# awslabs/flowgger

Hardware: AMD Instinct MI355X
Metric: log lines/sec (RFC5424, 256B avg) at 1/2/4/8 MI355X; achieved HBM GB/s (higher is better)
Workload: dtype u8

## Files before the change

### flowgger_amd/_lib.py

```python
from __future__ import annotations

import ctypes as C
from pathlib import Path

import os

_HERE = Path(__file__).resolve().parent
_ALT = os.environ.get("FLOWGGER_AMD_LIB") or ""
if _ALT and (Path(_ALT).name != _ALT or not _ALT.startswith("libfg_hip") or not _ALT.endswith(".so")):
    raise RuntimeError(f"FLOWGGER_AMD_LIB={_ALT!r}: only a bare libfg_hip*.so file name beside flowgger_amd/_lib.py is accepted")
LIB_PATH = _HERE / (_ALT or ("libfg_hip_prof.so" if os.environ.get("FLOWGGER_AMD_PROF_LIB") else "libfg_hip.so"))

FG_ABI_VERSION = 4
FG_RFC5424, FG_LTSV, FG_GELF, FG_RFC3164, FG_CAPNP = 0, 1, 2, 3, 4
FG_EF_VAL_ESC, FG_EF_NAME_ESC, FG_EF_SUFFIX, FG_EF_NAME_VERBATIM = 1, 2, 4, 8
FG_FRAME_NONE, FG_FRAME_LINE, FG_FRAME_NUL, FG_FRAME_SYSLEN = 0, 1, 2, 3
FG_SYSLEN_CLEAN, FG_SYSLEN_TAIL, FG_SYSLEN_BAD_LEN, FG_SYSLEN_LONG_PREFIX = 0, 1, 2, 3
FG_SYSLEN_MAX_PREFIX = 24
FG_UDP_RAW, FG_UDP_ZLIB, FG_UDP_GZIP, FG_UDP_BAD_ZLIB, FG_UDP_BAD_GZIP, FG_UDP_BAD_UTF8, FG_UDP_TOO_LARGE = range(7)
FG_UDP_DEFAULT_MAX_INFLATED = 65_527 * 5
FG_ST_OVERFLOW, FG_ST_BAD_UTF8 = 0xFE, 0xFD
FG_F_LTSV_NOVALUE = 128
FG_OK, FG_ERR_ARG, FG_ERR_HIP, FG_ERR_NO_DEVICE, FG_ERR_ENT_OVERFLOW, FG_ERR_UNSUPPORTED, FG_ERR_NOMEM = 0, -1, -2, -3, -4, -5, -6
FG_YEAR_NOW = -2147483648
# ... 45 lines not shown

class fg_launch_opts(C.Structure):
    _fields_ = [("lines_per_group", C.c_uint32), ("tile_cap", C.c_uint32), ("waves_per_cu", C.c_uint32),
                ("gelf_lds_budget", C.c_uint32), ("gelf_window_kib", C.c_uint32), ("flags", C.c_uint32), ("chunk_lines", C.c_uint32), ("ent_chunk", C.c_uint32), ("fused_look", C.c_uint32), ("fused_ext", C.c_uint32)]


FG_LO_GELF_GENERIC, FG_LO_TRANSCODE_ONE_PIECE, FG_LO_NO_HEAD, FG_LO_FORCE_HEAD, FG_LO_SD_WALK, FG_LO_SD_PAIRS, FG_LO_NO_ZERO_COPY, FG_LO_FRAME_KERNEL_UPLOAD = 1, 2, 4, 8, 16, 32, 64, 128
FG_LO_FRAME_CLASSIC = 256
FG_LO_STATIC_CHUNKS = 512
FG_LO_FRAME_SELFTEST_STALL = 1024
FG_LO_NO_TAPER = 2048
FG_LO_TAPER_1 = 4096
FG_LO_TAPER_2 = 8192
FG_LO_NO_FUSED_FRAMING = 16384
FG_LO_RFC3164_REGROUP, FG_LO_RFC3164_NO_REGROUP = 32768, 65536
FG_PATH_DECODE_ZERO_COPY, FG_PATH_DECODE_SLICED, FG_PATH_FRAME_FUSED, FG_PATH_FRAME_SLICED, FG_PATH_FRAME_ONE_PIECE = 1, 2, 3, 4, 5
FG_PATH_FRAME_SYSLEN_DEVICE, FG_PATH_FRAME_SYSLEN_HOST = 6, 7
FG_LO_RESERVED = 0x40000000


class fg_transcoded(C.Structure):
    _fields_ = [("out", C.c_void_p), ("out_bytes", C.c_uint64), ("out_offsets", C.c_void_p), ("meta", C.c_void_p),
                ("enc_status", C.c_void_p), ("frame_offsets", C.c_void_p), ("n", C.c_uint64), ("consumed", C.c_uint64)]


class fg_tz_table(C.Structure):
    _fields_ = [("n_zones", C.c_uint32), ("names", C.POINTER(C.c_char_p)), ("zone_first", C.c_void_p), ("utc_start", C.c_void_p),
                ("utc_offset", C.c_void_p)]


# ... 96 lines not shown
```

### flowgger_amd/csrc/fg_pipeline.hpp

```cpp
#pragma once
#include "fg_device.hpp"
#include "fg_plan_policy.hpp"
#include "fg_wave.hpp"

namespace fg {

using u32x4 = unsigned int __attribute__((ext_vector_type(4)));

__device__ __forceinline__ uint32_t eq_flags(uint32_t x, uint32_t pat) {
    uint32_t s = ((x & 0x7F7F7F7Fu) ^ pat) + 0x7F7F7F7Fu;
    return ~(s | x) & 0x80808080u;
}
__device__ __forceinline__ uint32_t range_flags(uint32_t x) {
    uint32_t l = x & 0x7F7F7F7Fu;
    uint32_t ge33 = l + 0x5F5F5F5Fu;
    uint32_t le126 = l + 0x01010101u;
    return ge33 & ~le126 & ~x & 0x80808080u;
}
__device__ __forceinline__ uint32_t ctrl_flags(uint32_t x) {
    uint32_t ge32 = (x & 0x7F7F7F7Fu) + 0x60606060u;
    return ~(ge32 | x) & 0x80808080u;
}
__device__ __forceinline__ uint32_t gather16(uint32_t f0, uint32_t f1, uint32_t f2, uint32_t f3) {
    uint32_t lo = __builtin_amdgcn_udot4(f1, 0x80402010u, __builtin_amdgcn_udot4(f0, 0x08040201u, 0u, false), false);
// ... 237 lines not shown
    return make_uint4(v.x, v.y, v.z, v.w);
#else
    return *p;
#endif
}

template <class F, class = void>
struct tail_batch { static constexpr int value = 4; };
template <class F>
struct tail_batch<F, decltype((void)F::kTailBatch)> { static constexpr int value = F::kTailBatch; };

template <class F, class = void>
struct defer_row_store { static constexpr bool value = true; };
template <class F>
struct defer_row_store<F, decltype((void)F::kDeferRowStore)> { static constexpr bool value = F::kDeferRowStore; };

constexpr uint32_t kHeadCap = 1024;
template <class F, class = void>
struct head_cap { static constexpr uint32_t value = kHeadCap; };
template <class F>
struct head_cap<F, decltype((void)F::kHeadBytes)> { static constexpr uint32_t value = F::kHeadBytes; };

template <int NB, bool PROF, class F, bool HEAD = false>
__device__ __forceinline__ void persistent_loop(const uint8_t* __restrict__ bytes, const uint64_t* __restrict__ offsets,
                                                uint64_t n, const DevTables& t, uint32_t tile_cap, uint32_t L, uint64_t chunk_lines,
                                                unsigned long long* prof, uint64_t* stash_base, F& fmt, FrameArgs fr) {
    static_assert(!HEAD || F::kClasses <= 1, "HEAD staging classifies one stage-A byte class at most");
    const uint64_t kChunkLines = chunk_lines;
    extern __shared__ __attribute__((aligned(16))) uint8_t smem[];
    uint16_t* bm16 = reinterpret_cast<uint16_t*>(smem + tile_cap + 64u);
// ... 281 lines not shown
                if (HEAD && e1 != o1) {
                    l2 = 0u;
                    if (e1 - o0 >= 1u) l2 = byte_at(e1 - 1);
                    if (e1 - o0 >= 2u) l2 |= byte_at(e1 - 2) << 8;
                }
            }
            GroupCtx c{bytes, smem, bm16, o0, e1, a0, span, valid, li, (ablate & 8u) ? nullptr : stash, ablate, ent_state, PROF ? prof + 6 : nullptr};
            c.tile_cap = tile_cap;
            if constexpr (HEAD) {
                const uint32_t al = (uint32_t)(o0 & 15ull), len = (uint32_t)(e1 - o0);
                c.tbase = tb + al;
                c.tlen = st == 0u ? 0u : (st - al < len ? st - al : len);
                c.last2 = l2;
            }
            pend = fmt.decode(c, t);
            if (fr.line_bad && valid && fr.line_bad[li]) {
                pend.meta = FG_ST_BAD_UTF8 | (0xFFu << 8) | (0xFFu << 16);
                pend.ts = 0.0;
#pragma unroll
                for (int k = 0; k < 6; ++k) pend.span[k] = fg_span{0, FG_NONE};
                pend.count = 0;
            }
            pend_li = li;
            pend_valid = valid;
#if defined(FG_ROW64_AB) && FG_ROW64_AB == 2
            pend_p = p;
            pend_nl = nl;
            if (!HEAD && defer_row_store<F>::value) {
                uint4 w[4];
                pack_row64(pend, w);
// ... 36 lines not shown
    }
#if defined(FG_ROW64_AB) && FG_ROW64_AB == 2
    if (!HEAD && defer_row_store<F>::value) {
        if (pend_valid && !(ablate & 1u)) {
            uint4* g = reinterpret_cast<uint4*>(t.meta) + pend_li * 4u;
            g[0] = pw0, g[1] = pw1, g[2] = pw2, g[3] = pw3;
        }
    } else if (pend_valid && !(ablate & 1u)) {
        store_row64_lane(t, pend_li, pend);
    }
#elif defined(FG_ROW64_AB)
    if (pend_valid && !(ablate & 1u)) store_row64_lane(t, pend_li, pend);
#else
    if (pend_valid && !(ablate & 1u)) store_row(t, pend_li, pend);
#endif
    if (PROF && lane == 0) {
        atomicAdd(&prof[0], (unsigned long long)acc0);
        atomicAdd(&prof[1], (unsigned long long)acc1);
        atomicAdd(&prof[2], (unsigned long long)acc2);
        atomicAdd(&prof[3], (unsigned long long)acc3);
        atomicAdd(&prof[4], (unsigned long long)iters);
    }
}

}

#include <cstdio>
#include <cstdlib>

namespace fg {
// ... 130 lines not shown
```

### flowgger_amd/csrc/fg_plan_policy.hpp

```cpp
#pragma once
#include <stdint.h>

#include "../../include/fg_hip.h"

#if defined(__HIPCC__)
#define FG_POLICY_HD __host__ __device__
#else
#define FG_POLICY_HD
#endif

namespace fg {

constexpr uint32_t kNoTaper = 0xFFFFFFFFu;

FG_POLICY_HD inline void chunk_range(uint64_t c, uint64_t chunk, uint32_t t0, uint32_t t1, uint32_t t2, uint64_t n, uint64_t* lo,
                                     uint64_t* hi) {
    uint64_t base = 0, first = 0, sz = chunk;
    if (c >= t0) {
        base = (uint64_t)t0 * sz, first = t0, sz >>= 1;
        if (c >= t1) {
            base += (uint64_t)(t1 - t0) * sz, first = t1, sz >>= 1;
            if (c >= t2) base += (uint64_t)(t2 - t1) * sz, first = t2, sz >>= 1;
        }
    }
// ... 63 lines not shown
        uint32_t levels = 0;
        while (levels < taper && (chunk >> (levels + 1u)) >= g) ++levels;
        if (m >= 1u && levels >= 1u && p.chunks + 4u * m < 0xFFFFFFF0ull) {
            const uint64_t t0 = (n - m * chunk) / chunk;
            p.taper[0] = (uint32_t)t0;
            if (levels >= 2u) p.taper[1] = (uint32_t)(t0 + m);
            if (levels >= 3u) p.taper[2] = (uint32_t)(t0 + 2u * m);
            p.chunks = count_chunks(chunk, p.taper, n);
        }
    }
    p.blocks = (uint32_t)(blocks > p.chunks ? p.chunks : blocks);
    p.tickets = tickets;
    return p;
}

inline uint32_t entry_chunk(uint64_t ent_cap, uint32_t blocks, uint64_t n, const fg_launch_opts& lo, uint32_t shares = 1) {
    if (lo.ent_chunk == 1u) return 0u;
    if (lo.ent_chunk >= 2u) return lo.ent_chunk;
    const uint64_t waves = blocks ? blocks : 1u;
    const uint64_t budget = ent_cap / (shares ? shares : 1u);
    uint64_t c = budget / (16ull * waves);
    if (c > 4096u) c = 4096u;
    if (budget / (4ull * waves) < 256u) return 0u;
    if (c < 256u) c = 256u;
    const uint64_t per_wave = (n + waves - 1u) / waves * 8ull;
    if (c > per_wave) c = per_wave;
    if (c < 256u) c = 256u;
    return (uint32_t)c;
}

// ... 2 lines not shown
```

### flowgger_amd/csrc/fg_rfc5424.hip

```cpp
#include <cstdio>
#include <cstdlib>

#include "fg_fused.hpp"
#include "fg_sd2.hpp"
#include "fg_tsfast.hpp"

namespace fg {

enum : uint32_t {
    E_OK = 0,
    E_BOM = 1,
    E_BRACKETS = 2,
    E_INVPRI = 3,
    E_NOVER = 4,
    E_BADVER = 5,
    E_NOTS = 6,
    E_BADTS = 7,
    E_NOHOST = 8,
    E_NOAPP = 9,
    E_NOPROC = 10,
    E_NOMSGID = 11,
    E_NODATA = 12,
    E_NOMSG = 13,
    E_MALFORMED = 14,
// ... 244 lines not shown
    for (int k = 0; k < 9; ++k) r[k] = __builtin_amdgcn_alignbyte(hdr[k + 2], hdr[k + 1], s);
    return fast_rfc3339_core(r, L, [&](uint32_t pos, uint32_t* z0, uint32_t* z1) { load8(T, a + pos, z0, z1); }, out);
}

__device__ __forceinline__ uint32_t take_space(uint64_t& lo, uint64_t& hi, uint32_t none, uint32_t& found) {
    const bool in_lo = lo != 0, in_hi = hi != 0;
    const uint32_t p = in_lo ? (uint32_t)__builtin_ctzll(lo) : in_hi ? 64u + (uint32_t)__builtin_ctzll(hi) : none;
    const uint64_t lo2 = lo & (lo - 1ull), hi2 = hi & (hi - 1ull);
    hi = in_lo ? hi : hi2;
    lo = lo2;
    found += (in_lo || in_hi) ? 1u : 0u;
    return p;
}

constexpr uint32_t kNoLastByte = 0xFFFFFFFFu;
__device__ __forceinline__ Fast parse_line_fast(const Tile& T, uint32_t base, uint32_t len, Row& r, uint32_t last_byte = kNoLastByte) {
    Fast f;
    uint32_t l0 = last_byte, l1;
    if (last_byte == kNoLastByte) load8(T, base + (len ? len - 1u : 0u), &l0, &l1);
    uint32_t hdr[33];
    {
        const uint32_t d = base >> 2, sft = base & 3u;
        uint32_t raw[34];
#pragma unroll
        for (int k = 0; k < 34; ++k) raw[k] = T.w[d + k];
#pragma unroll
        for (int k = 0; k < 33; ++k) hdr[k] = __builtin_amdgcn_alignbyte(raw[k + 1], raw[k], sft);
    }
    const uint32_t h0 = hdr[0], h1 = hdr[1];

    const uint32_t c1 = ((h0 >> 8) & 0xFFu) - '0', c2 = ((h0 >> 16) & 0xFFu) - '0', c3 = (h0 >> 24) - '0';
    const bool d2 = c2 <= 9u, d3 = d2 && c3 <= 9u;
    const uint32_t nd = 1u + (d2 ? 1u : 0u) + (d3 ? 1u : 0u);
    uint32_t pri = c1;
// ... 45 lines not shown
    r.len[S_APP] = s3 - s2 - 1u;
    r.off[S_PROC] = s3 + 1u;
    r.len[S_PROC] = s4 - s3 - 1u;
    r.off[S_MSGID] = s4 + 1u;
    r.len[S_MSGID] = s5 - s4 - 1u;
    const uint32_t d0 = s5 + 1u;
    f.d0 = d0;
    f.rest = found < 5u ? E_NOHOST + found : d0 >= len ? E_NOMSG : E_OK;

    uint32_t m0, m1;
    load8(T, base + (d0 < len ? d0 : 0u), &m0, &m1);
    const uint32_t c = m0 & 0xFFu;
    f.c7 = c;
    const bool live = !f.no_ts && f.rest == E_OK;
    f.route |= (live && c != '-') ? R_TAIL : 0u;
    const uint32_t last = l0 & 0xFFu;
    const bool end_plain = last > 0x20u && last < 0x80u;
    f.e = len;
    const uint32_t cA = (m0 >> 8) & 0xFFu, cB = (m0 >> 16) & 0xFFu;
    const uint32_t s = d0 + 1u;
    const bool one_sp = s + 1u < len && cA == ' ' && cB > 0x20u && cB < 0x80u;
    const bool no_sp = s < len && cA > 0x20u && cA < 0x80u;
    f.s = one_sp ? s + 1u : s;
    f.route |= (live && c == '-' && !(end_plain && (one_sp || no_sp))) ? R_TRIM : 0u;
    return f;
}

struct QuoteClass {
    static __device__ __forceinline__ uint32_t mask16(const uint4& v) {
        const uint32_t Q = 0x22222222u, B = 0x5C5C5C5Cu;
        return gather16(eq_flags(v.x, Q) | eq_flags(v.x, B), eq_flags(v.y, Q) | eq_flags(v.y, B),
                        eq_flags(v.z, Q) | eq_flags(v.z, B), eq_flags(v.w, Q) | eq_flags(v.w, B));
    }
};
__device__ __forceinline__ bool is_sd_name_char(uint32_t c) {
    return (c - 33u) <= 93u && c != '"' && c != '=' && c != ']';
}
struct WinMasks {
    uint32_t space;
// ... 213 lines not shown
    if (st != E_OK) {
        r.n_ent = 0;
        if (walk_len < len) return false;
        r.status = st;
        return true;
    }
    if (!finish_sd_tail(T, base, len, walk_len, last2, msg_at, r, gbytes, o0)) {
        r.n_ent = 0;
        return false;
    }
    return true;
}

constexpr uint32_t kShortSdTail = 64;

template <bool HEAD, bool SDX = false, bool PROF = false>
struct Rfc5424FormatT {
    static constexpr uint32_t kClasses = 0;
    static __device__ __forceinline__ void classify_store(const uint4&, uint16_t*, uint32_t, uint32_t, uint32_t) {}
    unsigned long long* pacc = nullptr;

    __device__ __forceinline__ RowOut decode(const GroupCtx& c, const DevTables& t) const {
    const uint8_t* __restrict__ bytes = c.bytes;
    const uint8_t* smem = c.smem;
    uint16_t* bm16 = c.bm16;
    const uint64_t o0 = c.o0, o1 = c.o1, a0 = c.a0;
    const uint32_t span = c.span, ablate = c.ablate;
    const bool valid = c.valid;
    uint64_t* stash = c.stash;
    const uint32_t lane = threadIdx.x;
    Row r;
#pragma unroll
// ... 8 lines not shown
    const uint32_t base = HEAD ? c.tbase : (uint32_t)(o0 - a0);
    bool from_global = false;
    uint32_t* tile_w = reinterpret_cast<uint32_t*>(const_cast<uint8_t*>(smem));
    bool rec_ok = false;
    Tile T{reinterpret_cast<const uint32_t*>(smem), reinterpret_cast<const uint32_t*>(bm16)};
    uint64_t pc[10] = {0, 0, 0, 0, 0, 0, 0, 0, 0, 0}, tk = PROF ? wv::clock() : 0;
    auto tick = [&](int k) {
        if (PROF) {
            const uint64_t now = wv::clock();
            pc[k] += now - tk;
            tk = now;
        }
    };
    uint32_t route = 0;
    Fast f{};
    if (valid) {
        route = R_GENERIC;
        if (in_tile || head_only) {
            f = parse_line_fast(T, base, len, r, HEAD ? (len ? (c.last2 & 0xFFu) : 0u) : kNoLastByte);
            route = f.route;
            if (!(route & R_GENERIC)) {
                if (route & R_TS_SLOW) {
                    LdsReader rd(T.w, base);
                    bool ok = parse_rfc3339(rd, f.t0, f.te, &r.ts);
                    r.status = f.no_ts ? E_NOTS : ok ? f.rest : E_BADTS;
                } else {
                    r.status = f.no_ts ? E_NOTS : f.ts_ok ? f.rest : E_BADTS;
                }
            }
        }
    }
    const bool sd_any = valid && !(route & R_GENERIC) && (route & R_TAIL) && r.status == E_OK && f.c7 == '[';
    const uint64_t sd_ballot = __ballot(sd_any);
    const bool group_has_sd = __any(sd_any && len - f.d0 > kShortSdTail) || __popcll(sd_ballot) > 4;
    const bool sd_lane = sd_any && group_has_sd;
    tick(0);
    sd2::Lds SL{};
    sd2::LineIn sin{false, 0u, 0u, 0u, false};
    sd2::LineOut slo{false, 0u, false, E_OK, 0u, 0u, 0u};
    bool sd2_ran = false;
    if constexpr (SDX) {
        if (group_has_sd) {
            const uint32_t stride16 = c.tile_cap / 16u + 16u;
            SL = sd2::carve(smem, bm16, c.tile_cap, reinterpret_cast<uint8_t*>(bm16 + 2u * stride16));
            __syncthreads();
            const bool chain = sd2::classify_tile(SL, span);
            __syncthreads();
            tick(1);
            sin = sd2::LineIn{sd_lane && (in_tile || head_only), base, f.d0, walk_len, in_tile};
            if (!chain) {
                slo = sd2::group_walk<PROF>(SL, span, sin, pc);
                sd2_ran = true;
            }
            tk = PROF ? wv::clock() : 0;
        }
    } else if (group_has_sd) {
        __syncthreads();
        rebuild_bitmap<QuoteClass>(smem, bm16, span >> 4);
        __syncthreads();
    }
    bool redo = false;
    bool coop = false;
    if (valid) {
        if (!(route & R_GENERIC)) {
            if (r.status == E_OK) {
                if (SDX && sd_lane) {
                    redo = !slo.handled;
                    if (slo.handled) {
                        r.data0 = f.d0;
                        if (slo.status != E_OK) {
                            r.status = slo.status;
                        } else {
                            r.n_ent = slo.n_ent;
                            redo = !finish_sd_tail(T, base, len, walk_len, c.last2, slo.msg_at, r, bytes, o0);
                        }
                    }
                } else if (sd_lane) {
                    redo = !parse_tail_sd_tile(T, base, f.d0, len, walk_len, c.last2, r, t, stash ? tile_w : nullptr, &rec_ok, bytes, o0);
// ... 113 lines not shown
                GlobalReader rd(reinterpret_cast<const uint32_t*>(bytes), o0);
                sd_walk<true>(rd, r.data0, len, &msg_at, &cnt, t, first);
            }
        }
    }

    tick(8);
    RowOut o;
    const bool ok = r.status == E_OK;
    o.meta = r.status | (r.facility << 8) | (r.severity << 16) | (r.flags << 24);
    o.ts = ok ? r.ts : 0.0;
#pragma unroll
    for (int k = 0; k < 6; ++k) o.span[k] = ok ? fg_span{r.off[k], r.len[k]} : fg_span{0, FG_NONE};
    o.first = first;
    o.count = r.n_ent;
    if constexpr (HEAD) {
        unsigned long long todo = __ballot(coop);
        while (todo) {
            const int src = (int)__builtin_ctzll(todo);
            todo &= todo - 1ull;
            auto rl64 = [&](uint64_t x) -> uint64_t {
                return (uint64_t)(uint32_t)__builtin_amdgcn_readlane((int)(uint32_t)x, src) |
                       ((uint64_t)(uint32_t)__builtin_amdgcn_readlane((int)(uint32_t)(x >> 32), src) << 32);
            };
            const uint64_t ro0 = rl64(o0), ro1 = rl64(o1), rli = rl64(c.li);
            const uint64_t ra0 = ro0 & ~15ull;
            const uint32_t rspan = (uint32_t)((ro1 - ra0 + 15ull) & ~15ull);
            __syncthreads();
            {
                __amdgpu_buffer_rsrc_t rsrc = __builtin_amdgcn_make_buffer_rsrc(const_cast<uint8_t*>(bytes + ra0), (short)0, (int)rspan, 0x00020000);
// ... 26 lines not shown
            if ((int)lane == src) {
                o.meta = g_meta;
                o.ts = __builtin_bit_cast(double, (unsigned long long)((uint64_t)g_ts0 | ((uint64_t)g_ts1 << 32)));
#pragma unroll
                for (int k = 0; k < 6; ++k) o.span[k] = fg_span{g_off[k], g_len[k]};
                o.first = g_first;
                o.count = g_count;
            }
        }
    }
    tick(9);
    if (PROF && pacc && lane == 0)
        for (int k = 0; k < 10; ++k) pacc[k] += (unsigned long long)pc[k];
    return o;
    }
};

using Rfc5424Format = Rfc5424FormatT<false>;

template <int NB, bool PROF, bool HEAD = false, bool SDX = false>
__global__ __launch_bounds__(kWave, 2) void k_rfc5424(const uint8_t* __restrict__ bytes,
                                                     const uint64_t* __restrict__ offsets, uint64_t n, DevTables t,
                                                     uint32_t tile_cap, uint32_t L, uint64_t groups,
                                                     unsigned long long* prof, uint64_t* stash_base, FrameArgs fr) {
    Rfc5424FormatT<HEAD, SDX, PROF> fmt;
    if constexpr (PROF) {
        __shared__ unsigned long long pacc[10];
        if (threadIdx.x < 10) pacc[threadIdx.x] = 0ull;
        fmt.pacc = pacc;
        __syncthreads();
        persistent_loop<NB, PROF, Rfc5424FormatT<HEAD, SDX, PROF>, HEAD>(bytes, offsets, n, t, tile_cap, L, groups, prof, stash_base, fmt, fr);
        __syncthreads();
        if (prof && threadIdx.x < 10) atomicAdd(&prof[6 + threadIdx.x], pacc[threadIdx.x]);
    } else if constexpr (SDX) {
        __shared__ DevTables t_lds;
        if (threadIdx.x == 0) t_lds = t;
        __syncthreads();
        persistent_loop<NB, PROF, Rfc5424FormatT<HEAD, SDX, PROF>, HEAD>(bytes, offsets, n, t_lds, tile_cap, L, groups, prof, stash_base, fmt, fr);
    } else {
        persistent_loop<NB, PROF, Rfc5424FormatT<HEAD, SDX, PROF>, HEAD>(bytes, offsets, n, t, tile_cap, L, groups, prof, stash_base, fmt, fr);
    }
}

template <int NB, bool SDX>
__global__ __launch_bounds__(kWave, 2) void k_rfc5424_fused(const uint8_t* __restrict__ bytes, DevTables t, uint32_t tile_cap, uint32_t L,
                                                           uint64_t* stash_base, FusedArgs fa, uint32_t strip) {
    Rfc5424FormatT<false, SDX, false> fmt;
    __shared__ DevTables t_lds;
    __shared__ FusedArgs fa_lds;
    if (threadIdx.x == 0) {
        t_lds = t;
        fa_lds = fa;
    }
    __syncthreads();
    fused_loop<NB>(bytes, t_lds, tile_cap, L, fmt, fa_lds, strip, stash_base);
}

}

extern "C" uint64_t fg_stash_bytes(uint32_t blocks) {
    return (uint64_t)blocks * fg::kStashEntries * fg::kStashWords * fg::kWave * sizeof(uint64_t);
}

constexpr uint32_t kShortLineTile = 17408;
static_assert(kShortLineTile + 64u + (kShortLineTile / 16u + 16u) * 2u <= 160u * 1024u / 8u, "eight waves per CU");
static_assert(kShortLineTile + 1024u + 64u + ((kShortLineTile + 1024u) / 16u + 16u) * 2u > 160u * 1024u / 8u, "the largest such tile");

extern "C" int fg_launch_rfc5424(const uint8_t* d_bytes, const uint64_t* d_offsets, uint64_t n, const fg::DevTables* t,
                                 uint64_t avg_len, hipStream_t stream, uint64_t* stash, uint32_t stash_blocks, uint32_t strip,
                                 const uint8_t* line_bad, const fg_launch_opts* lo, fg::TicketSlot* tk) {
    if (n == 0) return 0;
    fg::LaunchPlan p;
    const bool head = (lo->flags & FG_LO_FORCE_HEAD) || (avg_len >= 768u && !(lo->flags & FG_LO_NO_HEAD));
    const bool sdx = (lo->flags & FG_LO_SD_PAIRS) || (avg_len >= 320u && !(lo->flags & FG_LO_SD_WALK));
    const uint64_t plan_len = head ? (avg_len < fg::kHeadCap ? avg_len : fg::kHeadCap) : avg_len;
    const uint32_t sb = stash ? stash_blocks : 0u;
    int prc;
    if (sdx)
        prc = head ? fg::plan_launch(fg::k_rfc5424<fg::kWindowKiB, false, true, true>, n, plan_len, 0u, 36864u, sb, &p, *lo,
                                     fg::PlanFormat().classes(2u).lds_tile(fg::sd2::extra_bytes).tile(12288u).chunk(128u).tickets_from(4u))
                   : fg::plan_launch(fg::k_rfc5424<fg::kWindowKiB, false, false, true>, n, plan_len, 0u, 36864u, sb, &p, *lo,
                                     fg::PlanFormat().classes(2u).lds_tile(fg::sd2::extra_bytes).tile(12288u).chunk(128u).tickets_from(4u));
    else
        prc = head ? fg::plan_launch(fg::k_rfc5424<fg::kWindowKiB, false, true>, n, plan_len, 0u, 57344u, sb, &p, *lo)
                   : fg::plan_launch(fg::k_rfc5424<fg::kWindowKiB, false>, n, plan_len, 0u, 57344u, sb, &p, *lo,
                                     fg::PlanFormat().tickets_from(20u).taper_levels(0u).tile(avg_len < 320u ? kShortLineTile : 0u));
    if (prc) return -1;
    if (stash_blocks == 0) stash = nullptr;
    dim3 grid(p.blocks), block(fg::kWave);
    fg::FrameArgs fr{strip, line_bad};
    fg::take_tickets(&fr, tk, p);
    fg::DevTables tt = *t;
    tt.alloc_chunk = fg::entry_chunk(tt.ent_cap, p.blocks, n, *lo, tt.shares);
    unsigned long long* const no_prof = nullptr;
#define FG_LAUNCH_5424(PROF_, HEAD_, SDX_, prof_ptr)                                                                                       \
    hipLaunchKernelGGL((fg::k_rfc5424<fg::kWindowKiB, PROF_, HEAD_, SDX_>), grid, block, p.lds, stream, d_bytes, d_offsets, n, tt, p.tile, p.L, \
                       p.chunk, prof_ptr, stash, fr)
#if defined(FG_PROF_BUILD)
    if (fg::prof_requested()) {
        fg::ProfRun pr;
        if (!pr.begin(stream)) return -1;
        if (sdx) {
            if (head) FG_LAUNCH_5424(true, true, true, pr.d);
            else FG_LAUNCH_5424(true, false, true, pr.d);
        } else {
            if (head) FG_LAUNCH_5424(true, true, false, pr.d);
            else FG_LAUNCH_5424(true, false, false, pr.d);
        }
        pr.end(stream, head ? (sdx ? "rfc5424 (head, pairs)" : "rfc5424 (head)") : (sdx ? "rfc5424 (pairs)" : "rfc5424"), p);
        return (int)hipGetLastError();
    }
#endif
    if (sdx) {
        if (head) FG_LAUNCH_5424(false, true, true, no_prof);
        else FG_LAUNCH_5424(false, false, true, no_prof);
    } else {
        if (head) FG_LAUNCH_5424(false, true, false, no_prof);
        else FG_LAUNCH_5424(false, false, false, no_prof);
    }
#undef FG_LAUNCH_5424
    return (int)hipGetLastError();
}

extern "C" int fg_launch_rfc5424_fused(const uint8_t* d_bytes, uint64_t nbytes, const fg::DevTables* t, const fg::FusedGeom* g, hipStream_t stream,
                                       uint64_t* stash, uint32_t stash_blocks, uint32_t strip, int final_, uint64_t* d_offsets, uint64_t cap,
                                       uint8_t* scratch, const fg_launch_opts* lo, unsigned long long** d_total) {
    if (nbytes == 0 || !g->ok) return -1;
    const bool sdx = g->variant == 1u;
    const uint32_t base_lds = g->tile + 64u + (g->tile / 16u + 16u) * 2u * (sdx ? 2u : 1u) + (sdx ? fg::sd2::extra_bytes(g->tile) : 0u);
    fg::FusedArgs fa{};
    uint32_t lds = 0, blocks = 0;
    if (stash_blocks == 0) stash = nullptr;
    const uint32_t delim = strip == FG_FRAME_LINE ? 0x0Au : 0u;
    const int prc = sdx ? fg::fused_prepare(fg::k_rfc5424_fused<12, true>, *g, base_lds, nbytes, final_, delim, d_offsets, cap, scratch,
                                            stash ? stash_blocks : 0u, *lo, stream, &fa, &lds, &blocks)
// ... 13 lines not shown
```

### flowgger_amd/decoder.py

```python
from __future__ import annotations

import ctypes as C
from typing import Iterable, List, Optional, Sequence, Tuple, Union

import numpy as np

from . import _lib as L
from .record import DecodeError, Record, parse_canonical
from .tables import DeviceTables, HostTables

_TYPE_IDS = {"string": L.FG_T_STRING, "bool": L.FG_T_BOOL, "f64": L.FG_T_F64, "i64": L.FG_T_I64, "u64": L.FG_T_U64}


def pack_lines(lines: Iterable[Union[str, bytes]]) -> Tuple[np.ndarray, np.ndarray]:
    bl = [ln.encode("utf-8", "surrogateescape") if isinstance(ln, str) else bytes(ln) for ln in lines]
    offsets = np.zeros(len(bl) + 1, np.uint64)
    if bl:
        offsets[1:] = np.cumsum([len(b) for b in bl], dtype=np.uint64)
    data = np.frombuffer(b"".join(bl), np.uint8).copy() if bl else np.zeros(0, np.uint8)
    return data, offsets


class Decoder:

# ... 8 lines not shown

    def _make_cfg(self, config: Optional[dict]):
        return None

    def clone_boxed(self) -> "Decoder":
        other = object.__new__(type(self))
        other._cfg = self._cfg
        other._keep = getattr(self, "_keep", None)
        other.device = self.device
        other._ctx = C.c_void_p()
        L.check(L.lib().fg_clone(self._ctx, C.byref(other._ctx)), "fg_clone")
        return other

    def set_launch_opts(self, lines_per_group: int = 0, tile_cap: int = 0, waves_per_cu: int = 0, gelf_lds_budget: int = 0,
                        gelf_window_kib: int = 0, gelf_generic: bool = False, transcode_one_piece: bool = False, chunk_lines: int = 0,
                        no_head: bool = False, force_head: bool = False, sd_walk: bool = False, sd_pairs: bool = False, no_zero_copy: bool = False, frame_kernel_upload: bool = False, frame_classic: bool = False, static_chunks: bool = False, frame_selftest_stall: bool = False, ent_chunk: int = 0, no_taper: bool = False, taper_levels: int = 0, no_fused_framing: bool = False, fused_look: int = 0, fused_ext: int = 0, rfc3164_regroup: int = 0) -> None:
        lo = L.fg_launch_opts(lines_per_group, tile_cap, waves_per_cu, gelf_lds_budget, gelf_window_kib,
                              (L.FG_LO_GELF_GENERIC if gelf_generic else 0) | (L.FG_LO_TRANSCODE_ONE_PIECE if transcode_one_piece else 0) |
                              (L.FG_LO_NO_HEAD if no_head else 0) | (L.FG_LO_FORCE_HEAD if force_head else 0) |
                              (L.FG_LO_SD_WALK if sd_walk else 0) | (L.FG_LO_SD_PAIRS if sd_pairs else 0) | (L.FG_LO_NO_ZERO_COPY if no_zero_copy else 0) | (L.FG_LO_FRAME_KERNEL_UPLOAD if frame_kernel_upload else 0) | (L.FG_LO_FRAME_CLASSIC if frame_classic else 0) | (L.FG_LO_STATIC_CHUNKS if static_chunks else 0) | (L.FG_LO_FRAME_SELFTEST_STALL if frame_selftest_stall else 0) | (L.FG_LO_NO_TAPER if no_taper else 0) | (L.FG_LO_TAPER_1 if taper_levels & 1 else 0) | (L.FG_LO_TAPER_2 if taper_levels & 2 else 0) | (L.FG_LO_NO_FUSED_FRAMING if no_fused_framing else 0) | (L.FG_LO_RFC3164_REGROUP if rfc3164_regroup == 1 else L.FG_LO_RFC3164_NO_REGROUP if rfc3164_regroup == 2 else 0),
                              chunk_lines, ent_chunk, fused_look, fused_ext)
        L.check(L.lib().fg_set_launch_opts(self._ctx, C.byref(lo)), "fg_set_launch_opts")

    def close(self) -> None:
        if getattr(self, "_ctx", None) is not None and self._ctx.value:
            L.lib().fg_destroy(self._ctx)
            self._ctx = C.c_void_p()

    def __del__(self):
        try:
            self.close()
        except Exception:
            pass

    def decode(self, line: Union[str, bytes]) -> Record:
# ... 415 lines not shown
```

### include/fg_hip.h

```cpp
#ifndef FG_HIP_H
#define FG_HIP_H
#include <stdint.h>

#ifdef __cplusplus
extern "C" {
#endif

#define FG_ABI_VERSION 4

typedef enum fg_format { FG_RFC5424 = 0, FG_LTSV = 1, FG_GELF = 2, FG_RFC3164 = 3, FG_CAPNP = 4 } fg_format;

enum {
    FG_OK = 0,
    FG_ERR_ARG = -1,
    FG_ERR_HIP = -2,
    FG_ERR_NO_DEVICE = -3,
    FG_ERR_ENT_OVERFLOW = -4,
    FG_ERR_UNSUPPORTED = -5,
    FG_ERR_NOMEM = -6
};

enum {
    FG_T_STRING = 0, FG_T_BOOL = 1, FG_T_F64 = 2, FG_T_I64 = 3, FG_T_U64 = 4, FG_T_NULL = 5,
    FG_T_SDID = 6
// ... 116 lines not shown
    FG_LO_NO_HEAD = 4,
    FG_LO_FORCE_HEAD = 8,
    FG_LO_SD_WALK = 16,
    FG_LO_SD_PAIRS = 32,
    FG_LO_NO_ZERO_COPY = 64,
    FG_LO_FRAME_KERNEL_UPLOAD = 128,
    FG_LO_FRAME_CLASSIC = 256,
    FG_LO_STATIC_CHUNKS = 512,
    FG_LO_FRAME_SELFTEST_STALL = 1024,
    FG_LO_NO_TAPER = 2048,
    FG_LO_TAPER_1 = 4096,
    FG_LO_TAPER_2 = 8192,
    FG_LO_NO_FUSED_FRAMING = 16384,
    FG_LO_RFC3164_REGROUP = 32768,
    FG_LO_RFC3164_NO_REGROUP = 65536,
    FG_LO_RESERVED = 0x40000000
};

int fg_create(int device, const fg_cfg* cfg, fg_ctx** out);
int fg_clone(const fg_ctx* ctx, fg_ctx** out);
void fg_destroy(fg_ctx* ctx);
int fg_last_hip_error(const fg_ctx* ctx);
int fg_set_launch_opts(fg_ctx* ctx, const fg_launch_opts* opts);
int fg_set_rfc3164(fg_ctx* ctx, const fg_rfc3164_cfg* cfg);

#define FG_TABLE_ARRAYS 15
int fg_tables_layout(uint64_t n, uint64_t ent_cap, uint64_t sizes[FG_TABLE_ARRAYS]);

int fg_decode_batch_device(fg_ctx* ctx, fg_format fmt, const uint8_t* d_bytes, uint64_t nbytes,
                           const uint64_t* d_offsets, uint64_t n, const fg_tables* tables,
// ... 142 lines not shown
```

### integration/rust/fg-hip-sys/src/lib.rs

```rust
#![allow(non_camel_case_types, non_upper_case_globals, non_snake_case, dead_code)]
use std::os::raw::{c_char, c_int, c_void};

pub const FG_ABI_VERSION: c_int = 4;
pub type fg_format = c_int;
pub const FG_RFC5424: fg_format = 0;
pub const FG_LTSV: fg_format = 1;
pub const FG_GELF: fg_format = 2;
pub const FG_RFC3164: fg_format = 3;
pub const FG_CAPNP: fg_format = 4;

pub const FG_OK: c_int = 0;
pub const FG_ERR_ARG: c_int = -1;
pub const FG_ERR_HIP: c_int = -2;
pub const FG_ERR_NO_DEVICE: c_int = -3;
pub const FG_ERR_ENT_OVERFLOW: c_int = -4;
pub const FG_ERR_UNSUPPORTED: c_int = -5;
pub const FG_ERR_NOMEM: c_int = -6;

pub const FG_T_STRING: c_int = 0;
pub const FG_T_BOOL: c_int = 1;
pub const FG_T_F64: c_int = 2;
pub const FG_T_I64: c_int = 3;
pub const FG_T_U64: c_int = 4;
pub const FG_T_NULL: c_int = 5;
// ... 117 lines not shown
pub const FG_LO_NO_HEAD: c_int = 4;
pub const FG_LO_FORCE_HEAD: c_int = 8;
pub const FG_LO_SD_WALK: c_int = 16;
pub const FG_LO_SD_PAIRS: c_int = 32;
pub const FG_LO_NO_ZERO_COPY: c_int = 64;
pub const FG_LO_FRAME_KERNEL_UPLOAD: c_int = 128;
pub const FG_LO_FRAME_CLASSIC: c_int = 256;
pub const FG_LO_STATIC_CHUNKS: c_int = 512;
pub const FG_LO_FRAME_SELFTEST_STALL: c_int = 1024;
pub const FG_LO_NO_TAPER: c_int = 2048;
pub const FG_LO_TAPER_1: c_int = 4096;
pub const FG_LO_TAPER_2: c_int = 8192;
pub const FG_LO_NO_FUSED_FRAMING: c_int = 16384;
pub const FG_LO_RFC3164_REGROUP: c_int = 32768;
pub const FG_LO_RFC3164_NO_REGROUP: c_int = 65536;
pub const FG_LO_RESERVED: c_int = 1073741824;

pub const FG_TABLE_ARRAYS: c_int = 15;
pub type fg_udp_status = c_int;
pub const FG_UDP_RAW: fg_udp_status = 0;
pub const FG_UDP_ZLIB: fg_udp_status = 1;
pub const FG_UDP_GZIP: fg_udp_status = 2;
pub const FG_UDP_BAD_ZLIB: fg_udp_status = 3;
pub const FG_UDP_BAD_GZIP: fg_udp_status = 4;
pub const FG_UDP_BAD_UTF8: fg_udp_status = 5;
pub const FG_UDP_TOO_LARGE: fg_udp_status = 6;

pub const FG_UDP_DEFAULT_MAX_INFLATED: u32 = 0x4FFD3;
pub const FG_UDP_MAX_MAX_INFLATED: u32 = 0x7FFFFFF0;
pub const FG_PATH_DECODE_ZERO_COPY: c_int = 1;
// ... 315 lines not shown
```

Measured before the change: 17.05 billion.

## Park rare RFC5424 lines in an LDS list and drain them wave-wide

Adds a parking instantiation of the RFC5424 kernel. When a wave holds only a few lines (at most four) that need the slow generic, tail, trim or slow-timestamp path, their indices go into a 64-entry shared-memory list and are later parsed in a batch, one line per lane, so rare lines stop serializing the whole wave through divergent slow paths. It also adds a TRIM8 fast path that checks up to 8 trailing and leading blank bytes, so fewer lines take the trim route. The parking kernel is picked by default when groups per block are high enough. The cost is extra LDS, more ballots and syncs, and a second plan_launch call on the host.

```diff
diff --git a/flowgger_amd/_lib.py b/flowgger_amd/_lib.py
--- a/flowgger_amd/_lib.py
+++ b/flowgger_amd/_lib.py
@@ -83,6 +83,7 @@
 FG_LO_TAPER_2 = 8192
 FG_LO_NO_FUSED_FRAMING = 16384
 FG_LO_RFC3164_REGROUP, FG_LO_RFC3164_NO_REGROUP = 32768, 65536
+FG_LO_RFC5424_PARK, FG_LO_RFC5424_NO_PARK = 131072, 262144
 FG_PATH_DECODE_ZERO_COPY, FG_PATH_DECODE_SLICED, FG_PATH_FRAME_FUSED, FG_PATH_FRAME_SLICED, FG_PATH_FRAME_ONE_PIECE = 1, 2, 3, 4, 5
 FG_PATH_FRAME_SYSLEN_DEVICE, FG_PATH_FRAME_SYSLEN_HOST = 6, 7
 FG_LO_RESERVED = 0x40000000
diff --git a/flowgger_amd/csrc/fg_park.hpp b/flowgger_amd/csrc/fg_park.hpp
--- /dev/null
+++ b/flowgger_amd/csrc/fg_park.hpp
@@ -0,0 +1,39 @@
+#pragma once
+#include "fg_wave.hpp"
+
+namespace fg {
+namespace park {
+
+constexpr uint32_t kCap = 64;
+constexpr uint32_t kMaxRare = 4;
+constexpr uint32_t kListBytes = kCap * 8u;
+
+struct List {
+    uint64_t* slot = nullptr;
+    uint32_t count = 0;
+};
+
+FG_WV bool parks(uint64_t rare) { return rare != 0ull && wv::popc64(rare) <= kMaxRare; }
+
+FG_WV uint32_t append(List& l, uint64_t rare, uint64_t line) {
+    const uint32_t me = wv::lane();
+    if ((rare >> me) & 1ull) l.slot[l.count + wv::mbcnt(rare)] = line;
+    const uint32_t n = wv::popc64(rare);
+    l.count += n;
+    return n;
+}
+
+FG_WV bool must_flush(const List& l) { return l.count + kMaxRare > kCap; }
+
+FG_WV bool drain(List& l, uint64_t* line) {
+    const uint32_t me = wv::lane();
+    wv::sync();
+    const bool mine = me < l.count;
+    *line = mine ? l.slot[me] : 0ull;
+    wv::sync();
+    l.count = 0u;
+    return mine;
+}
+
+}
+}
diff --git a/flowgger_amd/csrc/fg_pipeline.hpp b/flowgger_amd/csrc/fg_pipeline.hpp
--- a/flowgger_amd/csrc/fg_pipeline.hpp
+++ b/flowgger_amd/csrc/fg_pipeline.hpp
@@ -275,6 +275,11 @@
 struct defer_row_store { static constexpr bool value = true; };
 template <class F>
 struct defer_row_store<F, decltype((void)F::kDeferRowStore)> { static constexpr bool value = F::kDeferRowStore; };
+
+template <class F, class = void>
+struct parks_lines { static constexpr bool value = false; };
+template <class F>
+struct parks_lines<F, decltype((void)F::kParkLines)> { static constexpr bool value = F::kParkLines; };
 
 constexpr uint32_t kHeadCap = 1024;
 template <class F, class = void>
@@ -586,6 +591,9 @@
                 c.last2 = l2;
             }
             pend = fmt.decode(c, t);
+            if constexpr (parks_lines<F>::value) {
+                if (fmt.park_must_flush()) fmt.flush_parked(bytes, offsets, t, fr.strip, fr.line_bad, ent_state, ablate);
+            }
             if (fr.line_bad && valid && fr.line_bad[li]) {
                 pend.meta = FG_ST_BAD_UTF8 | (0xFFu << 8) | (0xFFu << 16);
                 pend.ts = 0.0;
@@ -652,6 +660,7 @@
 #else
     if (pend_valid && !(ablate & 1u)) store_row(t, pend_li, pend);
 #endif
+    if constexpr (parks_lines<F>::value) fmt.flush_parked(bytes, offsets, t, fr.strip, fr.line_bad, ent_state, ablate);
     if (PROF && lane == 0) {
         atomicAdd(&prof[0], (unsigned long long)acc0);
         atomicAdd(&prof[1], (unsigned long long)acc1);
diff --git a/flowgger_amd/csrc/fg_plan_policy.hpp b/flowgger_amd/csrc/fg_plan_policy.hpp
--- a/flowgger_amd/csrc/fg_plan_policy.hpp
+++ b/flowgger_amd/csrc/fg_plan_policy.hpp
@@ -101,6 +101,13 @@
     return p;
 }
 
+constexpr uint32_t kParkMinGroupsPerWave = 16;
+inline bool park_lines(uint64_t groups, uint32_t blocks, const fg_launch_opts& lo) {
+    if (lo.flags & FG_LO_RFC5424_NO_PARK) return false;
+    if (lo.flags & FG_LO_RFC5424_PARK) return true;
+    return groups >= (uint64_t)kParkMinGroupsPerWave * (blocks ? blocks : 1u);
+}
+
 inline uint32_t entry_chunk(uint64_t ent_cap, uint32_t blocks, uint64_t n, const fg_launch_opts& lo, uint32_t shares = 1) {
     if (lo.ent_chunk == 1u) return 0u;
     if (lo.ent_chunk >= 2u) return lo.ent_chunk;
diff --git a/flowgger_amd/csrc/fg_rfc5424.hip b/flowgger_amd/csrc/fg_rfc5424.hip
--- a/flowgger_amd/csrc/fg_rfc5424.hip
+++ b/flowgger_amd/csrc/fg_rfc5424.hip
@@ -2,6 +2,7 @@
 #include <cstdlib>
 
 #include "fg_fused.hpp"
+#include "fg_park.hpp"
 #include "fg_sd2.hpp"
 #include "fg_tsfast.hpp"
 
@@ -282,10 +283,11 @@
 }
 
 constexpr uint32_t kNoLastByte = 0xFFFFFFFFu;
+template <bool TRIM8 = false>
 __device__ __forceinline__ Fast parse_line_fast(const Tile& T, uint32_t base, uint32_t len, Row& r, uint32_t last_byte = kNoLastByte) {
     Fast f;
-    uint32_t l0 = last_byte, l1;
-    if (last_byte == kNoLastByte) load8(T, base + (len ? len - 1u : 0u), &l0, &l1);
+    uint32_t l0 = last_byte, l1 = 0;
+    if (last_byte == kNoLastByte) load8(T, base + (TRIM8 ? (len >= 8u ? len - 8u : 0u) : (len ? len - 1u : 0u)), &l0, &l1);
     uint32_t hdr[33];
     {
         const uint32_t d = base >> 2, sft = base & 3u;
@@ -361,15 +363,40 @@
     f.c7 = c;
     const bool live = !f.no_ts && f.rest == E_OK;
     f.route |= (live && c != '-') ? R_TAIL : 0u;
-    const uint32_t last = l0 & 0xFFu;
-    const bool end_plain = last > 0x20u && last < 0x80u;
-    f.e = len;
-    const uint32_t cA = (m0 >> 8) & 0xFFu, cB = (m0 >> 16) & 0xFFu;
-    const uint32_t s = d0 + 1u;
-    const bool one_sp = s + 1u < len && cA == ' ' && cB > 0x20u && cB < 0x80u;
-    const bool no_sp = s < len && cA > 0x20u && cA < 0x80u;
-    f.s = one_sp ? s + 1u : s;
-    f.route |= (live && c == '-' && !(end_plain && (one_sp || no_sp))) ? R_TRIM : 0u;
+    if constexpr (TRIM8) {
+        auto nonblank = [](uint64_t v) -> uint64_t {
+            return ((uint64_t)(~eq_flags((uint32_t)(v >> 32), 0x20202020u) & 0x80808080u) << 32) | (~eq_flags((uint32_t)v, 0x20202020u) & 0x80808080u);
+        };
+        bool end_ok;
+        f.e = len;
+        if (last_byte == kNoLastByte) {
+            const uint64_t v = (((uint64_t)l1 << 32) | l0) << (len >= 8u ? 0u : ((8u - len) & 7u) * 8u);
+            const uint64_t nb = nonblank(v);
+            const uint32_t j = nb ? (uint32_t)__builtin_clzll(nb) >> 3 : 8u;
+            const uint32_t cE = (uint32_t)((v << ((j & 7u) * 8u)) >> 56);
+            end_ok = j < 8u && cE > 0x20u && cE < 0x80u;
+            f.e = len - (end_ok ? j : 0u);
+        } else {
+            end_ok = last_byte > 0x20u && last_byte < 0x80u;
+        }
+        const uint32_t s = d0 + 1u;
+        const uint64_t mv = (((uint64_t)m1 << 32) | m0) >> 8;
+        const uint32_t jS = (uint32_t)__builtin_ctzll(nonblank(mv)) >> 3;
+        const uint32_t cS = (uint32_t)(mv >> (jS * 8u)) & 0xFFu;
+        const bool start_ok = s + jS < len && cS > 0x20u && cS < 0x80u;
+        f.s = start_ok ? s + jS : s;
+        f.route |= (live && c == '-' && !(end_ok && start_ok)) ? R_TRIM : 0u;
+    } else {
+        const uint32_t last = l0 & 0xFFu;
+        const bool end_plain = last > 0x20u && last < 0x80u;
+        f.e = len;
+        const uint32_t cA = (m0 >> 8) & 0xFFu, cB = (m0 >> 16) & 0xFFu;
+        const uint32_t s = d0 + 1u;
+        const bool one_sp = s + 1u < len && cA == ' ' && cB > 0x20u && cB < 0x80u;
+        const bool no_sp = s < len && cA > 0x20u && cA < 0x80u;
+        f.s = one_sp ? s + 1u : s;
+        f.route |= (live && c == '-' && !(end_plain && (one_sp || no_sp))) ? R_TRIM : 0u;
+    }
     return f;
 }
 
@@ -613,8 +640,11 @@
 
 constexpr uint32_t kShortSdTail = 64;
 
-template <bool HEAD, bool SDX = false, bool PROF = false>
+template <bool HEAD, bool SDX = false, bool PROF = false, bool PARK = false, bool TRIM8 = false>
 struct Rfc5424FormatT {
+    static_assert(!PARK || (!HEAD && !SDX), "parking: the whole-line kernel without the pair-parallel walk only");
+    static constexpr bool kParkLines = PARK;
+    mutable park::List pk;
     static constexpr uint32_t kClasses = 0;
     static __device__ __forceinline__ void classify_store(const uint4&, uint16_t*, uint32_t, uint32_t, uint32_t) {}
     unsigned long long* pacc = nullptr;
@@ -653,23 +683,49 @@
     };
     uint32_t route = 0;
     Fast f{};
-    if (valid) {
-        route = R_GENERIC;
-        if (in_tile || head_only) {
-            f = parse_line_fast(T, base, len, r, HEAD ? (len ? (c.last2 & 0xFFu) : 0u) : kNoLastByte);
-            route = f.route;
-            if (!(route & R_GENERIC)) {
-                if (route & R_TS_SLOW) {
-                    LdsReader rd(T.w, base);
-                    bool ok = parse_rfc3339(rd, f.t0, f.te, &r.ts);
-                    r.status = f.no_ts ? E_NOTS : ok ? f.rest : E_BADTS;
-                } else {
-                    r.status = f.no_ts ? E_NOTS : f.ts_ok ? f.rest : E_BADTS;
-                }
-            }
-        }
-    }
-    const bool sd_any = valid && !(route & R_GENERIC) && (route & R_TAIL) && r.status == E_OK && f.c7 == '[';
+    bool parked = false;
+    if constexpr (!PARK) {
+        if (valid) {
+            route = R_GENERIC;
+            if (in_tile || head_only) {
+                f = parse_line_fast<TRIM8>(T, base, len, r, HEAD ? (len ? (c.last2 & 0xFFu) : 0u) : kNoLastByte);
+                route = f.route;
+                if (!(route & R_GENERIC)) {
+                    if (route & R_TS_SLOW) {
+                        LdsReader rd(T.w, base);
+                        bool ok = parse_rfc3339(rd, f.t0, f.te, &r.ts);
+                        r.status = f.no_ts ? E_NOTS : ok ? f.rest : E_BADTS;
+                    } else {
+                        r.status = f.no_ts ? E_NOTS : f.ts_ok ? f.rest : E_BADTS;
+                    }
+                }
+            }
+        }
+    } else {
+        if (valid) {
+            route = R_GENERIC;
+            if (in_tile) {
+                f = parse_line_fast<TRIM8>(T, base, len, r, kNoLastByte);
+                route = f.route;
+            }
+        }
+        const bool rare = valid && (route & (R_GENERIC | R_TAIL | R_TRIM | R_TS_SLOW)) != 0u;
+        const uint64_t rare_m = wv::ballot(rare);
+        if (park::parks(rare_m)) {
+            park::append(pk, rare_m, c.li);
+            parked = rare;
+        }
+        if (valid && !parked && in_tile && !(route & R_GENERIC)) {
+            if (route & R_TS_SLOW) {
+                LdsReader rd(T.w, base);
+                bool ok = parse_rfc3339(rd, f.t0, f.te, &r.ts);
+                r.status = f.no_ts ? E_NOTS : ok ? f.rest : E_BADTS;
+            } else {
+                r.status = f.no_ts ? E_NOTS : f.ts_ok ? f.rest : E_BADTS;
+            }
+        }
+    }
+    const bool sd_any = valid && !parked && !(route & R_GENERIC) && (route & R_TAIL) && r.status == E_OK && f.c7 == '[';
     const uint64_t sd_ballot = __ballot(sd_any);
     const bool group_has_sd = __any(sd_any && len - f.d0 > kShortSdTail) || __popcll(sd_ballot) > 4;
     const bool sd_lane = sd_any && group_has_sd;
@@ -700,7 +756,7 @@
     }
     bool redo = false;
     bool coop = false;
-    if (valid) {
+    if (valid && !parked) {
         if (!(route & R_GENERIC)) {
             if (r.status == E_OK) {
                 if (SDX && sd_lane) {
@@ -844,6 +900,7 @@
     for (int k = 0; k < 6; ++k) o.span[k] = ok ? fg_span{r.off[k], r.len[k]} : fg_span{0, FG_NONE};
     o.first = first;
     o.count = r.n_ent;
+    if constexpr (PARK) o.skip = parked;
     if constexpr (HEAD) {
         unsigned long long todo = __ballot(coop);
         while (todo) {
@@ -900,31 +957,101 @@
         for (int k = 0; k < 10; ++k) pacc[k] += (unsigned long long)pc[k];
     return o;
     }
+
+    __device__ __forceinline__ bool park_must_flush() const { return PARK && park::must_flush(pk); }
+
+    __device__ __forceinline__ void flush_parked(const uint8_t* __restrict__ bytes, const uint64_t* __restrict__ offsets, const DevTables& t,
+                                                 uint32_t strip, const uint8_t* line_bad, uint32_t* ent_state, uint32_t ablate) const {
+        if constexpr (PARK) {
+            if (pk.count == 0u) return;
+            uint64_t li = 0;
+            const bool mine = park::drain(pk, &li);
+            Row r;
+#pragma unroll
+            for (int k = 0; k < 6; ++k) {
+                r.off[k] = 0;
+                r.len[k] = FG_NONE;
+            }
+            uint64_t o0 = 0;
+            uint32_t len = 0;
+            if (mine) {
+                o0 = offsets[li];
+                uint64_t e1 = offsets[li + 1];
+                if (strip != FG_FRAME_NONE && e1 > o0) {
+                    const uint32_t b1 = bytes[e1 - 1];
+                    if (strip == FG_FRAME_LINE) {
+                        if (b1 == '\n') {
+                            --e1;
+                            if (e1 > o0 && bytes[e1 - 1] == '\r') --e1;
+                        }
+                    } else if (b1 == 0u) {
+                        --e1;
+                    }
+                }
+                len = (uint32_t)(e1 - o0);
+                GlobalReader rd(reinterpret_cast<const uint32_t*>(bytes), o0);
+                parse_line_generic(rd, len, r, t);
+            }
+            const EntAlloc ea = alloc_entries_ex(t, r.n_ent, ent_state);
+            const uint32_t slot = (ea.overflow || ea.total == 0u) ? 0u : ea.s.at(ea.ex);
+            if (ea.overflow) {
+                r.status = FG_ST_OVERFLOW;
+                r.n_ent = 0;
+            }
+            const uint32_t first = r.n_ent != 0 ? slot : 0u;
+            if (r.n_ent != 0 && !(ablate & 4u)) {
+                uint32_t msg_at, cnt;
+                GlobalReader rd(reinterpret_cast<const uint32_t*>(bytes), o0);
+                sd_walk<true>(rd, r.data0, len, &msg_at, &cnt, t, first);
+            }
+            RowOut o;
+            const bool ok = r.status == E_OK;
+            o.meta = r.status | (r.facility << 8) | (r.severity << 16) | (r.flags << 24);
+            o.ts = ok ? r.ts : 0.0;
+#pragma unroll
+            for (int k = 0; k < 6; ++k) o.span[k] = ok ? fg_span{r.off[k], r.len[k]} : fg_span{0, FG_NONE};
+            o.first = first;
+            o.count = r.n_ent;
+            if (line_bad && mine && line_bad[li]) {
+                o.meta = FG_ST_BAD_UTF8 | (0xFFu << 8) | (0xFFu << 16);
+                o.ts = 0.0;
+#pragma unroll
+                for (int k = 0; k < 6; ++k) o.span[k] = fg_span{0, FG_NONE};
+                o.count = 0;
+            }
+            if (mine && !(ablate & 1u)) store_row(t, li, o);
+        }
+    }
 };
 
 using Rfc5424Format = Rfc5424FormatT<false>;
 
-template <int NB, bool PROF, bool HEAD = false, bool SDX = false>
+template <int NB, bool PROF, bool HEAD = false, bool SDX = false, bool PARK = false>
 __global__ __launch_bounds__(kWave, 2) void k_rfc5424(const uint8_t* __restrict__ bytes,
                                                      const uint64_t* __restrict__ offsets, uint64_t n, DevTables t,
                                                      uint32_t tile_cap, uint32_t L, uint64_t groups,
                                                      unsigned long long* prof, uint64_t* stash_base, FrameArgs fr) {
-    Rfc5424FormatT<HEAD, SDX, PROF> fmt;
+    using Fmt = Rfc5424FormatT<HEAD, SDX, PROF, PARK, !HEAD && !SDX>;
+    Fmt fmt;
+    if constexpr (PARK) {
+        __shared__ uint64_t park_list[park::kCap];
+        fmt.pk.slot = park_list;
+    }
     if constexpr (PROF) {
         __shared__ unsigned long long pacc[10];
         if (threadIdx.x < 10) pacc[threadIdx.x] = 0ull;
         fmt.pacc = pacc;
         __syncthreads();
-        persistent_loop<NB, PROF, Rfc5424FormatT<HEAD, SDX, PROF>, HEAD>(bytes, offsets, n, t, tile_cap, L, groups, prof, stash_base, fmt, fr);
+        persistent_loop<NB, PROF, Fmt, HEAD>(bytes, offsets, n, t, tile_cap, L, groups, prof, stash_base, fmt, fr);
         __syncthreads();
         if (prof && threadIdx.x < 10) atomicAdd(&prof[6 + threadIdx.x], pacc[threadIdx.x]);
     } else if constexpr (SDX) {
         __shared__ DevTables t_lds;
         if (threadIdx.x == 0) t_lds = t;
         __syncthreads();
-        persistent_loop<NB, PROF, Rfc5424FormatT<HEAD, SDX, PROF>, HEAD>(bytes, offsets, n, t_lds, tile_cap, L, groups, prof, stash_base, fmt, fr);
+        persistent_loop<NB, PROF, Fmt, HEAD>(bytes, offsets, n, t_lds, tile_cap, L, groups, prof, stash_base, fmt, fr);
     } else {
-        persistent_loop<NB, PROF, Rfc5424FormatT<HEAD, SDX, PROF>, HEAD>(bytes, offsets, n, t, tile_cap, L, groups, prof, stash_base, fmt, fr);
+        persistent_loop<NB, PROF, Fmt, HEAD>(bytes, offsets, n, t, tile_cap, L, groups, prof, stash_base, fmt, fr);
     }
 }
 
@@ -950,6 +1077,8 @@
 
 constexpr uint32_t kShortLineTile = 17408;
 static_assert(kShortLineTile + 64u + (kShortLineTile / 16u + 16u) * 2u <= 160u * 1024u / 8u, "eight waves per CU");
+static_assert(kShortLineTile + 64u + (kShortLineTile / 16u + 16u) * 2u + fg::park::kListBytes <= 160u * 1024u / 8u,
+              "eight waves per CU with the pending list of the parking instantiation (static LDS)");
 static_assert(kShortLineTile + 1024u + 64u + ((kShortLineTile + 1024u) / 16u + 16u) * 2u > 160u * 1024u / 8u, "the largest such tile");
 
 extern "C" int fg_launch_rfc5424(const uint8_t* d_bytes, const uint64_t* d_offsets, uint64_t n, const fg::DevTables* t,
@@ -972,6 +1101,15 @@
                    : fg::plan_launch(fg::k_rfc5424<fg::kWindowKiB, false>, n, plan_len, 0u, 57344u, sb, &p, *lo,
                                      fg::PlanFormat().tickets_from(20u).taper_levels(0u).tile(avg_len < 320u ? kShortLineTile : 0u));
     if (prc) return -1;
+    bool park = !head && !sdx && fg::park_lines(p.groups, p.blocks, *lo);
+    if (park) {
+        fg::LaunchPlan pp;
+        if (fg::plan_launch(fg::k_rfc5424<fg::kWindowKiB, false, false, false, true>, n, plan_len, 0u, 57344u, sb, &pp, *lo,
+                            fg::PlanFormat().tickets_from(20u).taper_levels(0u).tile(avg_len < 320u ? kShortLineTile : 0u)) == 0)
+            p = pp;
+        else
+            park = false;
+    }
     if (stash_blocks == 0) stash = nullptr;
     dim3 grid(p.blocks), block(fg::kWave);
     fg::FrameArgs fr{strip, line_bad};
@@ -979,9 +1117,10 @@
     fg::DevTables tt = *t;
     tt.alloc_chunk = fg::entry_chunk(tt.ent_cap, p.blocks, n, *lo, tt.shares);
     unsigned long long* const no_prof = nullptr;
-#define FG_LAUNCH_5424(PROF_, HEAD_, SDX_, prof_ptr)                                                                                       \
-    hipLaunchKernelGGL((fg::k_rfc5424<fg::kWindowKiB, PROF_, HEAD_, SDX_>), grid, block, p.lds, stream, d_bytes, d_offsets, n, tt, p.tile, p.L, \
+#define FG_LAUNCH_5424_P(PROF_, HEAD_, SDX_, PARK_, prof_ptr)                                                                                      \
+    hipLaunchKernelGGL((fg::k_rfc5424<fg::kWindowKiB, PROF_, HEAD_, SDX_, PARK_>), grid, block, p.lds, stream, d_bytes, d_offsets, n, tt, p.tile, p.L, \
                        p.chunk, prof_ptr, stash, fr)
+#define FG_LAUNCH_5424(PROF_, HEAD_, SDX_, prof_ptr) FG_LAUNCH_5424_P(PROF_, HEAD_, SDX_, false, prof_ptr)
 #if defined(FG_PROF_BUILD)
     if (fg::prof_requested()) {
         fg::ProfRun pr;
@@ -991,9 +1130,10 @@
             else FG_LAUNCH_5424(true, false, true, pr.d);
         } else {
             if (head) FG_LAUNCH_5424(true, true, false, pr.d);
+            else if (park) FG_LAUNCH_5424_P(true, false, false, true, pr.d);
             else FG_LAUNCH_5424(true, false, false, pr.d);
         }
-        pr.end(stream, head ? (sdx ? "rfc5424 (head, pairs)" : "rfc5424 (head)") : (sdx ? "rfc5424 (pairs)" : "rfc5424"), p);
+        pr.end(stream, head ? (sdx ? "rfc5424 (head, pairs)" : "rfc5424 (head)") : (sdx ? "rfc5424 (pairs)" : park ? "rfc5424 (park)" : "rfc5424"), p);
         return (int)hipGetLastError();
     }
 #endif
@@ -1002,9 +1142,11 @@
         else FG_LAUNCH_5424(false, false, true, no_prof);
     } else {
         if (head) FG_LAUNCH_5424(false, true, false, no_prof);
+        else if (park) FG_LAUNCH_5424_P(false, false, false, true, no_prof);
         else FG_LAUNCH_5424(false, false, false, no_prof);
     }
 #undef FG_LAUNCH_5424
+#undef FG_LAUNCH_5424_P
     return (int)hipGetLastError();
 }
 
diff --git a/flowgger_amd/decoder.py b/flowgger_amd/decoder.py
--- a/flowgger_amd/decoder.py
+++ b/flowgger_amd/decoder.py
@@ -46,11 +46,11 @@
 
     def set_launch_opts(self, lines_per_group: int = 0, tile_cap: int = 0, waves_per_cu: int = 0, gelf_lds_budget: int = 0,
                         gelf_window_kib: int = 0, gelf_generic: bool = False, transcode_one_piece: bool = False, chunk_lines: int = 0,
-                        no_head: bool = False, force_head: bool = False, sd_walk: bool = False, sd_pairs: bool = False, no_zero_copy: bool = False, frame_kernel_upload: bool = False, frame_classic: bool = False, static_chunks: bool = False, frame_selftest_stall: bool = False, ent_chunk: int = 0, no_taper: bool = False, taper_levels: int = 0, no_fused_framing: bool = False, fused_look: int = 0, fused_ext: int = 0, rfc3164_regroup: int = 0) -> None:
+                        no_head: bool = False, force_head: bool = False, sd_walk: bool = False, sd_pairs: bool = False, no_zero_copy: bool = False, frame_kernel_upload: bool = False, frame_classic: bool = False, static_chunks: bool = False, frame_selftest_stall: bool = False, ent_chunk: int = 0, no_taper: bool = False, taper_levels: int = 0, no_fused_framing: bool = False, fused_look: int = 0, fused_ext: int = 0, rfc3164_regroup: int = 0, park: bool = False, no_park: bool = False) -> None:
         lo = L.fg_launch_opts(lines_per_group, tile_cap, waves_per_cu, gelf_lds_budget, gelf_window_kib,
                               (L.FG_LO_GELF_GENERIC if gelf_generic else 0) | (L.FG_LO_TRANSCODE_ONE_PIECE if transcode_one_piece else 0) |
                               (L.FG_LO_NO_HEAD if no_head else 0) | (L.FG_LO_FORCE_HEAD if force_head else 0) |
-                              (L.FG_LO_SD_WALK if sd_walk else 0) | (L.FG_LO_SD_PAIRS if sd_pairs else 0) | (L.FG_LO_NO_ZERO_COPY if no_zero_copy else 0) | (L.FG_LO_FRAME_KERNEL_UPLOAD if frame_kernel_upload else 0) | (L.FG_LO_FRAME_CLASSIC if frame_classic else 0) | (L.FG_LO_STATIC_CHUNKS if static_chunks else 0) | (L.FG_LO_FRAME_SELFTEST_STALL if frame_selftest_stall else 0) | (L.FG_LO_NO_TAPER if no_taper else 0) | (L.FG_LO_TAPER_1 if taper_levels & 1 else 0) | (L.FG_LO_TAPER_2 if taper_levels & 2 else 0) | (L.FG_LO_NO_FUSED_FRAMING if no_fused_framing else 0) | (L.FG_LO_RFC3164_REGROUP if rfc3164_regroup == 1 else L.FG_LO_RFC3164_NO_REGROUP if rfc3164_regroup == 2 else 0),
+                              (L.FG_LO_SD_WALK if sd_walk else 0) | (L.FG_LO_SD_PAIRS if sd_pairs else 0) | (L.FG_LO_NO_ZERO_COPY if no_zero_copy else 0) | (L.FG_LO_FRAME_KERNEL_UPLOAD if frame_kernel_upload else 0) | (L.FG_LO_FRAME_CLASSIC if frame_classic else 0) | (L.FG_LO_STATIC_CHUNKS if static_chunks else 0) | (L.FG_LO_FRAME_SELFTEST_STALL if frame_selftest_stall else 0) | (L.FG_LO_NO_TAPER if no_taper else 0) | (L.FG_LO_TAPER_1 if taper_levels & 1 else 0) | (L.FG_LO_TAPER_2 if taper_levels & 2 else 0) | (L.FG_LO_NO_FUSED_FRAMING if no_fused_framing else 0) | (L.FG_LO_RFC3164_REGROUP if rfc3164_regroup == 1 else L.FG_LO_RFC3164_NO_REGROUP if rfc3164_regroup == 2 else 0) | (L.FG_LO_RFC5424_PARK if park else 0) | (L.FG_LO_RFC5424_NO_PARK if no_park else 0),
                               chunk_lines, ent_chunk, fused_look, fused_ext)
         L.check(L.lib().fg_set_launch_opts(self._ctx, C.byref(lo)), "fg_set_launch_opts")
 
diff --git a/include/fg_hip.h b/include/fg_hip.h
--- a/include/fg_hip.h
+++ b/include/fg_hip.h
@@ -154,6 +154,8 @@
     FG_LO_NO_FUSED_FRAMING = 16384,
     FG_LO_RFC3164_REGROUP = 32768,
     FG_LO_RFC3164_NO_REGROUP = 65536,
+    FG_LO_RFC5424_PARK = 131072,
+    FG_LO_RFC5424_NO_PARK = 262144,
     FG_LO_RESERVED = 0x40000000
 };
 
diff --git a/integration/rust/fg-hip-sys/src/lib.rs b/integration/rust/fg-hip-sys/src/lib.rs
--- a/integration/rust/fg-hip-sys/src/lib.rs
+++ b/integration/rust/fg-hip-sys/src/lib.rs
@@ -155,6 +155,8 @@
 pub const FG_LO_NO_FUSED_FRAMING: c_int = 16384;
 pub const FG_LO_RFC3164_REGROUP: c_int = 32768;
 pub const FG_LO_RFC3164_NO_REGROUP: c_int = 65536;
+pub const FG_LO_RFC5424_PARK: c_int = 131072;
+pub const FG_LO_RFC5424_NO_PARK: c_int = 262144;
 pub const FG_LO_RESERVED: c_int = 1073741824;
 
 pub const FG_TABLE_ARRAYS: c_int = 15;
```

Measured after the change: 15.29 billion. -10.3%, worse.
